# AgatheSenellart/MultiVae

Hardware: AMD Instinct MI355X
Metric: train samples/sec (ELBO step) MoPoE MnistSvhn K=10 (higher is better)
Workload: dtype f32 (error-corrected 2xfp16 / 3xbf16 products, fp32 accumulate); 1 GPU; MoPoE MnistSvhn (mnist MLP + svhn conv), K=10, per-device batch 512, latent_dim 20, Adam lr 1e-3, fwd+ELBO+bwd+optimizer; global_batch=512, K=10, parallelism=dp1, launch=hipGraph replay (fwd + bwd) + Adam

## Files before the change

include/mvk.h:

```cpp
#ifndef MVK_H
#define MVK_H

#include <stdint.h>

#ifdef __cplusplus
extern "C" {
#endif

#define MVK_OK 0
#define MVK_EINVAL (-1)
#define MVK_ELAUNCH (-2)

#define MVK_MAX_MODALITIES 8
#define MVK_MVAE_MAX_SUBSETS 32
#define MVK_IWAE_MAX_EXPERTS 32

#define MVK_DIST_NORMAL 0
#define MVK_DIST_LAPLACE 1
#define MVK_DIST_BERNOULLI 2
#define MVK_DIST_CATEGORICAL 3

#define MVK_ACT_NONE 0
#define MVK_ACT_RELU 1
#define MVK_ACT_SIGMOID 2
// ... 284 lines not shown

int mvk_nchw_to_nhwc(const float* src, float* dst, int n, int c, int h, int w, void* stream);
int mvk_nhwc_to_nchw(const float* src, float* dst, int n, int c, int h, int w, void* stream);

int mvk_poe_fwd(const float* mus, const float* lvs, int E, int64_t n, float eps, int stable, float* mu, float* lv,
                void* stream);
int mvk_poe_bwd(const float* mus, const float* lvs, int E, int64_t n, float eps, int stable, const float* gmu,
                const float* glv, float* dmus, float* dlvs, void* stream);
int mvk_kl_gauss_fwd(const float* mean, int64_t n_mean, const float* lv, int64_t n_lv, const float* pmean, int64_t n_pmean,
                     const float* plv, int64_t n_plv, int64_t rows, int L, float* kl, void* stream);
int mvk_kl_gauss_bwd(const float* mean, int64_t n_mean, const float* lv, int64_t n_lv, const float* pmean, int64_t n_pmean,
                     const float* plv, int64_t n_plv, int64_t rows, int L, const float* g, float* dmean, float* dlv,
                     float* dpmean, float* dplv, void* stream);
int mvk_logprob_fwd(const float* recon, const float* target, int64_t n, int64_t n_target, int dist, float scale, int C,
                    float eps, float* lp, void* stream);
int mvk_logprob_bwd(const float* recon, const float* target, int64_t n, int64_t n_target, int dist, float scale, int C,
                    float eps, const float* g, float* drecon, void* stream);

#define MVK_COPY_MAX 8
typedef struct {
  void* dst;
  const void* src;
  int64_t bytes;
} mvk_copy_desc;
int mvk_copy_batch(const mvk_copy_desc* descs, int n, void* stream);

int mvk_adam_step(float* p, const float* g, float* m, float* v, int64_t n, double lr, double beta1, double beta2,
                  double eps, double weight_decay, int step, double grad_scale, void* stream);
int mvk_adam_step_amsgrad(float* p, const float* g, float* m, float* v, float* vmax, int64_t n, double lr, double beta1,
                          double beta2, double eps, double weight_decay, int step, double grad_scale, void* stream);
int mvk_adam_step_fused(float* p, float* g, float* m, float* v, float* vmax, int64_t n, double lr, double beta1,
                        double beta2, double eps, double weight_decay, int step, double grad_scale, int zero_grad,
                        void* stream);
int mvk_adam_prepare(double* state, float* scalars, void* stream);
int mvk_adam_step_dev(float* p, float* g, float* m, float* v, float* vmax, int64_t n, const float* scalars, int zero_grad,
                      void* stream);
int mvk_adam_step_pub(float* p, float* g, float* m, float* v, float* vmax, int64_t n, double lr, double beta1, double beta2,
                      double eps, double weight_decay, int step, double grad_scale, int zero_grad, float* publish, void* stream);
int mvk_adam_identity(float* scalars, void* stream);

int mvk_heads_fwd(const float* X, const float* W0, const float* b0, float* Y0, const float* W1, const float* b1,
                  float* Y1, int M, int N, int K, int64_t w_sk, int64_t w_sn, void* stream);

int mvk_heads_bwd(const float* X, int x_act, const float* dY0, const float* dY1, const float* W0, const float* W1,
                  int64_t w_sk, int64_t w_sn, int flat_c, float* dX, float* dW0, float* dW1, float* db0, float* db1,
                  float* dbprev, int M, int N, int K, float* ws, int64_t ws_floats, void* stream);

int mvk_defer_begin(float* arena, int64_t arena_floats, const float* grad, int64_t grad_floats);
int mvk_defer_flush(void* stream);
int mvk_defer_end(void* stream);
int64_t mvk_defer_wanted(void);
int mvk_defer_pending(void);

int mvk_comm_id_bytes(void);
int mvk_comm_unique_id(void* id);
int mvk_comm_init(void** comm, int world, int rank, const void* id);
int mvk_comm_destroy(void* comm);
int mvk_allreduce_avg(float* buf, int64_t n, int nseg, void* comm, void* stream);
int mvk_comm_available(void);
int mvk_comm_size(void* comm, int* world, int* rank);
int mvk_allreduce_avg_ranges(float* buf, const int64_t* off, const int64_t* cnt, int nrange, int64_t seg_floats, void* comm,
                             void* stream);
int mvk_event_create(void** ev);
int mvk_event_destroy(void* ev);
int mvk_event_record(void* ev, int external, void* stream);
int mvk_stream_wait_event(void* stream, void* ev);

int mvk_dense16_ok(int M, int N, int K);
int mvk_dense16_pack(const float* W, int N, int K, void* nk_hi, void* nk_lo, float* nk_inv, void* kn_hi, void* kn_lo,
                     float* kn_inv, void* stream);
int mvk_dense16_first(const float* Z, const float* W, const float* bias, const float* z_amax, void* hi, void* lo, float* bound,
                      int M, int N, int K, int act, void* stream);
int mvk_dense16_fwd_nll_rows(int N);
int mvk_dense16_colsum_rows(int M);
int mvk_dense16_fwd_nll(const void* h_hi, const void* h_lo, const float* h_bound, const void* w_hi, const void* w_lo,
                        const float* w_inv, const float* bias, const float* X, int xrows, const float* x_amax, float scale,
                        float grad_weight, void* g_hi, void* g_lo, float* g_bound, float* rows_part, float* colsum_part, int M,
                        int N, int K, void* stream);
int mvk_dense16_bwd_data(const void* g_hi, const void* g_lo, const float* g_bound, const void* wt_hi, const void* wt_lo,
                         const float* wt_inv, const void* mask_hi, float* dA, float* db, float* ws, int64_t ws_floats, int M, int N,
                         int K, void* stream);
int mvk_dense16_wgrad(const void* g_hi, const void* g_lo, const float* g_bound, const void* h_hi, const void* h_lo,
                      const float* h_bound, const float* colsum_part, int cs_rows, float* dW, float* db, float* ws,
                      int64_t ws_floats, int M, int N, int K, void* stream);
int mvk_dense16_unsplit(const void* hi, const void* lo, const float* bound, const float* rowf, float rowf_scale, int rowf_tile,
                        int M, int N, float* out, void* stream);
void mvk_dense16_debug(int flags);
void mvk_dense16_debug_stamps(float* four_floats);

int mvk_nexus_aggregate_fwd(const float* const* msgs, const uint8_t* const* masks, const float* keep_in, const float* u,
                            float dropout_rate, int M, int B, int D, float* agg, float* keep_out, void* stream);
int mvk_nexus_aggregate_bwd(const float* keep, const float* g, int M, int B, int D, float* const* dmsgs, void* stream);

int mvk_nexus_top_nll_fwd(const float* const* z, const float* const* r, const uint8_t* const* masks, const int* D,
                          const float* gamma, const int* adapt, int M, int B, float* const* rows, float* q, float* s2,
                          float* work, void* stream);
int mvk_nexus_top_nll_bwd(const float* const* z, const float* const* r, const uint8_t* const* masks, const int* D,
                          const float* gamma, const int* adapt, int M, int B, const float* const* grows, const float* q,
                          const float* s2, float* work, float* const* dr, void* stream);

int mvk_prof_enable(void* device_slots, int nslots, int32_t* host_kinds, double* host_work);
int mvk_prof_count(void);
int mvk_prof_calibrate(void* device_ticks, int n, void* stream);
int mvk_prof_clock_khz(void);

void mvk_debug_set_phase_buffer(unsigned long long* device_counters);
// ... 7 lines not shown
```

multivae_amd/_lib.py:

```python
import ctypes as C
import os

import torch

_HERE = os.path.dirname(os.path.abspath(__file__))


_ALWAYS_READ = {"MVK_TUNE", "MVK_LIB_PATH", "MVK_DEFER_MB", "MVK_SYNC_DEBUG", "MVK_TRAINER_ALLOW_CPU", "MVK_CPU_THREADS",
                "MVK_BENCH_SAME_GPU", "MVK_FORCE_DIST", "MVK_DIST_BACKEND", "MVK_ADAM_ZERO", "MVK_RCCL", "MVK_BENCH_CHILD", "MVK_OVERLAP", "MVK_GRAPH_ADAM"}


def _warn_ignored_switches():
    if os.environ.get("MVK_TUNE") == "1":
        return
    ignored = sorted(k for k in os.environ if k.startswith("MVK_") and k not in _ALWAYS_READ)
    if ignored:
        import warnings

        warnings.warn(f"{', '.join(ignored)} set without MVK_TUNE=1: experiment switches are ignored unless MVK_TUNE=1 "
                      "(this process runs the shipped configuration)", RuntimeWarning, stacklevel=3)


_warn_ignored_switches()

# ... 70 lines not shown
    "mvk_loss_backward_seed": [C.POINTER(SeedDesc), _i, _p, _p],
    "mvk_f32_to_bf3": [_p, _i64, _p, _p],
    "mvk_bf3_to_f32": [_p, _i64, _p, _p],
    "mvk_conv4s2_small_up_fwd_nll": [_p, _p, _p, _p, _i, _f, _p, _p, _i, _i, _i, _i, _i, _i, _p],
    "mvk_conv4s2_small_up_fwd_nll_w": [_p, _p, _p, _p, _i, _f, _f, _p, _p, _i, _i, _i, _i, _i, _i, _p],
    "mvk_conv4s2_small_up_fwd_nll_s": [_p, _p, _p, _p, _i, _f, _f, _p, _p, _i, _i, _i, _i, _i, _i, _p, _p],
    "mvk_conv4s2_small_up_fwd_s": [_p, _p, _p, _p, _i, _i, _i, _i, _i, _i, _p, _p],
    "mvk_conv4s2_small_up_fwd_nll_sy": [_p, _p, _p, _p, _i, _f, _f, _p, _p, _i, _i, _i, _i, _i, _i, _p, _p, _p],
    "mvk_conv4s2_small_up_bwd_pre_s": [_p, _p, _p, _i, _p, _p, _p, _p, _p, _p, _i64, _i, _i, _i, _i, _i, _p, _p, _p, _p],
    "mvk_conv4s2_small_up_bwd_pre": [_p, _p, _p, _i, _p, _p, _p, _p, _p, _p, _i64, _i, _i, _i, _i, _i, _p],
    "mvk_conv3x3": [_p, _p, _p, _p, _i, _i, _i, _i, _i, _i, _p, _i, _p, _p, _i64, _p],
    "mvk_conv3x3_y": [_p, _p, _p, _p, _i, _i, _i, _i, _i, _i, _p, _i, _p, _p, _p, _i64, _p],
    "mvk_conv3x3_res": [_p, _p, _p, _p, _i, _i, _i, _i, _i, _i, _p, _i, _p, _f, _p, _i64, _p],
    "mvk_conv3x3_wgrad": [_p, _p, _p, _i, _i, _i, _i, _i, _p, _i64, _p],
    "mvk_conv3x3_f": [_p, _p, _p, _p, _i, _i, _i, _i, _i, _i, _p, _i, _p, _f, _p, _i, _f, _p, _i64, _p],
    "mvk_conv3x3_wgrad_f": [_p, _p, _p, _p, _i, _i, _i, _i, _i, _i, _f, _p, _i64, _p],
    "mvk_conv3x3_s": [_p, _p, _p, _p, _i, _i, _i, _i, _i, _i, _p, _i, _p, _f, _p, _i, _f, _p, _p, _p, _p, _i64, _p],
    "mvk_conv3x3_s2": [_p, _p, _p, _p, _p, _i, _i, _i, _i, _i, _i, _p, _f, _p, _p, _p, _p, _i64, _p],
    "mvk_conv3x3_s_part": [_p, _i, _i, _p, _p, _p, _i, _i, _i, _i, _i, _i, _p, _i, _p, _i, _i, _f, _p, _p, _p, _p],
    "mvk_amax": [_p, _i64, _p, _p],
    "mvk_conv4s2_wgrad_s": [_p, _p, _p, _i, _i, _i, _i, _i, _p, _p, _p, _i64, _p],
    "mvk_gemm_smallk_amax": [_p, _p, _p, _i, _i, _i, _i, _p, _i, _i, _p, _p],
    "mvk_conv4s2_small_up_bwd_pre_y": [_p, _p, _p, _i, _p, _p, _p, _p, _p, _p, _i64, _i, _i, _i, _i, _i, _p, _p],
    "mvk_conv4s2_down_s": [_p, _p, _p, _p, _i, _i, _i, _i, _i, _i, _p, _i, _p, _p, _p, _p, _p, _i64, _p, _p],
    "mvk_conv4s2_up_s": [_p, _p, _p, _p, _i, _i, _i, _i, _i, _i, _p, _i, _p, _p, _p, _p, _p, _i64, _p, _p],
    "mvk_conv3x3_wgrad_s": [_p, _p, _p, _p, _i, _i, _i, _i, _i, _i, _f, _p, _p, _p, _i64, _p],
    "mvk_avgpool3s2_fwd": [_p, _p, _i, _i, _i, _i, _p],
    "mvk_avgpool3s2_bwd": [_p, _p, _i, _i, _i, _i, _p],
    "mvk_upsample2_fwd": [_p, _p, _i, _i, _i, _i, _p],
    "mvk_upsample2_bwd": [_p, _p, _i, _i, _i, _i, _p],
    "mvk_axpby": [_p, _f, _p, _f, _i64, _i, _p, _p],
    "mvk_transpose_act": [_p, _p, _i, _i, _i, _i, _p, _i, _p],
    "mvk_probe_mfma_bf16": [_p, _i, _i, _p],
    "mvk_probe_stream_copy": [_p, _p, _i64, _p],
    "mvk_device_rng": [_p, _i64, _p, _i, _f, _f, _p],
    "mvk_conv4s2_wgrad": [_p, _p, _p, _i, _i, _i, _i, _i, _i, _p, _i, _p, _i64, _p],
    "mvk_conv4s2_wgrad_pair": [_p, _p, _p, _i, _i, _i, _i, _p, _p, _p, _i, _i, _i, _i, _i, _p, _i64, _p],
    "mvk_conv4s2_up_nchw_small": [_p, _p, _p, _p, _i, _i, _i, _i, _i, _i, _p],
    "mvk_conv4s2_small_up_fwd": [_p, _p, _p, _p, _i, _i, _i, _i, _i, _i, _p],
    "mvk_conv4s2_small_down_fwd": [_p, _p, _p, _p, _i, _i, _i, _i, _i, _i, _p],
    "mvk_conv4s2_small_down_fwd_wref": [_p, _p, _p, _p, _i, _i, _i, _i, _i, _i, _p],
    "mvk_conv4s2_small_up_bwd": [_p, _p, _i, _p, _i, _p, _p, _p, _p, _p, _p, _i64, _i, _i, _i, _i, _i, _p],
    "mvk_pack_unflatten_weight": [_p, _i, _i, _p, _p],
    "mvk_unflatten_wgrad": [_p, _p, _p, _i, _i, _i, _p, _i64, _p],
    "mvk_flatten_wgrad": [_p, _p, _p, _i, _i, _i, _p, _i64, _p],
    "mvk_nchw_to_nhwc": [_p, _p, _i, _i, _i, _i, _p],
    "mvk_nhwc_to_nchw": [_p, _p, _i, _i, _i, _i, _p],
    "mvk_adam_step": [_p, _p, _p, _p, _i64, _d, _d, _d, _d, _d, _i, _d, _p],
    "mvk_heads_fwd": [_p, _p, _p, _p, _p, _p, _p, _i, _i, _i, _i64, _i64, _p],
    "mvk_heads_bwd": [_p, _i, _p, _p, _p, _p, _i64, _i64, _i, _p, _p, _p, _p, _p, _p, _i, _i, _i, _p, _i64, _p],
    "mvk_defer_begin": [_p, _i64, _p, _i64],
    "mvk_defer_flush": [_p],
    "mvk_defer_end": [_p],
    "mvk_adam_step_amsgrad": [_p, _p, _p, _p, _p, _i64, _d, _d, _d, _d, _d, _i, _d, _p],
    "mvk_adam_step_fused": [_p, _p, _p, _p, _p, _i64, _d, _d, _d, _d, _d, _i, _d, _i, _p],
    "mvk_copy_batch": [C.POINTER(CopyDesc), _i, _p],
    "mvk_adam_prepare": [_p, _p, _p],
    "mvk_adam_step_pub": [_p, _p, _p, _p, _p, _i64, _d, _d, _d, _d, _d, _i, _d, _i, _p, _p],
    "mvk_adam_identity": [_p, _p],
    "mvk_adam_step_dev": [_p, _p, _p, _p, _p, _i64, _p, _i, _p],
    "mvk_mmvae_std_fwd": [_p, _i, _i, _i, _p, _p],
    "mvk_mmvae_std_bwd": [_p, _p, _p, _i, _i, _i, _p, _p],
    "mvk_mmvae_latent_fwd": [_p, _p, _p, _p, _p, _p, _i, _i, _i, _i, _i, _p, _p, _p, _p, _i, _p, _p],
    "mvk_mmvae_objective_fwd": [_p, _p, _p, _p, _i, _i, _i, _i, _p, _p, _p, _p, _p, _f, _p],
    "mvk_mmvae_latent_bwd": [_p, _p, _p, _p, _p, _p, _p, _p, _p, _p, _p, _i, _i, _i, _i, _i, _i, _p, _p, _p, _p, _i, _f, _p],
    "mvk_mmvaeplus_cross_latent_fwd": [_p, _p, _p, _i64, _i, _i, _i, _p, _p],
    "mvk_mmvaeplus_cross_latent_bwd": [_p, _p, _i64, _i, _i, _i, _p, _p, _p],
    "mvk_mvae_posterior_fwd": [_p, _p, _p, _i, _p, _i, _p, _i, _i, _p, _p, _p, _p, _p],
    "mvk_mvae_posterior_bwd": [_p, _p, _p, _i, _p, _i, _p, _p, _i, _i, _p, _p, _p, _p],
    "mvk_gauss_sample_kl_fwd": [_p, _p, _p, _i, _i, _i, _p, _p, _p],
    "mvk_gauss_sample_kl_bwd": [_p, _p, _p, _p, _p, _i, _i, _i, _p, _p, _p],
    "mvk_iwae_sample": [_p, _p, _p, _i, _i, _i, _i, _p, _p],
    "mvk_iwae_logw": [_p, _p, _i, _p, _p, _i, _p, _p, _i, _i, _i, _i, _p, _p],
    "mvk_iwae_reduce": [_p, _i, _i, _i, _p, _p],
    "mvk_poe_fwd": [_p, _p, _i, _i64, _f, _i, _p, _p, _p],
    "mvk_poe_bwd": [_p, _p, _i, _i64, _f, _i, _p, _p, _p, _p, _p],
    "mvk_kl_gauss_fwd": [_p, _i64, _p, _i64, _p, _i64, _p, _i64, _i64, _i, _p, _p],
    "mvk_kl_gauss_bwd": [_p, _i64, _p, _i64, _p, _i64, _p, _i64, _i64, _i, _p, _p, _p, _p, _p, _p],
    "mvk_logprob_fwd": [_p, _p, _i64, _i64, _i, _f, _i, _f, _p, _p],
    "mvk_logprob_bwd": [_p, _p, _i64, _i64, _i, _f, _i, _f, _p, _p, _p],
    "mvk_comm_unique_id": [_p],
    "mvk_comm_init": [C.POINTER(C.c_void_p), _i, _i, _p],
    "mvk_comm_destroy": [_p],
    "mvk_allreduce_avg": [_p, _i64, _i, _p, _p],
    "mvk_comm_size": [_p, C.POINTER(C.c_int), C.POINTER(C.c_int)],
    "mvk_allreduce_avg_ranges": [_p, C.POINTER(C.c_int64), C.POINTER(C.c_int64), _i, _i64, _p, _p],
    "mvk_event_create": [C.POINTER(C.c_void_p)],
    "mvk_event_destroy": [_p],
    "mvk_event_record": [_p, _i, _p],
    "mvk_stream_wait_event": [_p, _p],
    "mvk_dense16_pack": [_p, _i, _i, _p, _p, _p, _p, _p, _p, _p],
    "mvk_dense16_first": [_p, _p, _p, _p, _p, _p, _p, _i, _i, _i, _i, _p],
    "mvk_dense16_fwd_nll": [_p, _p, _p, _p, _p, _p, _p, _p, _i, _p, _f, _f, _p, _p, _p, _p, _p, _i, _i, _i, _p],
    "mvk_dense16_bwd_data": [_p, _p, _p, _p, _p, _p, _p, _p, _p, _p, _i64, _i, _i, _i, _p],
    "mvk_dense16_wgrad": [_p, _p, _p, _p, _p, _p, _p, _i, _p, _p, _p, _i64, _i, _i, _i, _p],
    "mvk_dense16_unsplit": [_p, _p, _p, _p, _f, _i, _i, _i, _p, _p],
    "mvk_nexus_aggregate_fwd": [_p, _p, _p, _p, _f, _i, _i, _i, _p, _p, _p],
    "mvk_nexus_aggregate_bwd": [_p, _p, _i, _i, _i, _p, _p],
    "mvk_nexus_top_nll_fwd": [_p, _p, _p, _p, _p, _p, _i, _i, _p, _p, _p, _p, _p],
    "mvk_nexus_top_nll_bwd": [_p, _p, _p, _p, _p, _p, _i, _i, _p, _p, _p, _p, _p, _p],
}

_lib = None


class MvkError(RuntimeError):
# ... 165 lines not shown
```

multivae_amd/csrc/igemm.hip:

```cpp
#include "igemm_bf.hpp"
#include <mutex>
#include <vector>

namespace mvk {
namespace {
struct DeferState {
  std::mutex mu;
  bool active = false;
  float* arena = nullptr;
  long long cap = 0, used = 0;
  long long wanted = 0;
  const char* g0 = nullptr;
  const char* g1 = nullptr;
  std::vector<DeferItem> items;
  std::vector<hipStream_t> streams;
  std::vector<hipEvent_t> events;
};
DeferState g_defer;

void defer_note_stream(hipStream_t s) {
  for (hipStream_t t : g_defer.streams)
    if (t == s) return;
  g_defer.streams.push_back(s);
}
// ... 93 lines not shown
      it.blk0 = blocks;
      T.it[T.n++] = defer_compact(it);
      const int per = (256 >> it.zl_bits) * (it.vec4 ? 4 : 1);
      blocks += (unsigned)(((long long)it.M * it.N + per - 1) / per);
    }
    hipLaunchKernelGGL(splitk_reduce_batch_kernel, dim3(blocks), dim3(256), 0, s, T);
    if (hipGetLastError() != hipSuccess) rc = MVK_ELAUNCH;
  }
  g_defer.items.clear();
  if (last)
    g_defer.used = 0;
  else
    defer_note_stream(s);
  return rc;
}

extern "C" int mvk_defer_flush(void* stream) {
  std::lock_guard<std::mutex> lock(mvk::g_defer.mu);
  if (!mvk::g_defer.active) return MVK_OK;
  return defer_flush_locked(mvk_stream(stream), false);
}

extern "C" int mvk_defer_end(void* stream) {
  std::lock_guard<std::mutex> lock(mvk::g_defer.mu);
  if (!mvk::g_defer.active) return MVK_OK;
  const int rc = defer_flush_locked(mvk_stream(stream), true);
  mvk::g_defer.active = false;
  return rc;
}

extern "C" int64_t mvk_defer_wanted(void) {
  std::lock_guard<std::mutex> lock(mvk::g_defer.mu);
  return (int64_t)mvk::g_defer.wanted;
}

extern "C" int mvk_defer_pending(void) {
  std::lock_guard<std::mutex> lock(mvk::g_defer.mu);
  return (int)mvk::g_defer.items.size();
}

#include <cstdlib>

namespace mvk {

template <int BM, int BN>
static int launch_cfg(const GemmDesc& d, int zdim, hipStream_t s) {
  dim3 grid((d.M + BM - 1) / BM, (d.N + BN - 1) / BN, zdim);
  hipLaunchKernelGGL((igemm_kernel<BM, BN>), grid, dim3(256), 0, s, d);
  MVK_CHECK_LAUNCH();
  return MVK_OK;
}

static thread_local int g_last_bm = 0;

template <int BM, int BN, int BKT, int AMODE, int BMODE, bool AACT>
static int launch_fast_cfg(const GemmDesc& d, int zdim, hipStream_t s) {
  g_last_bm = BM;
  dim3 grid((d.M + BM - 1) / BM, (d.N + BN - 1) / BN, zdim);
  hipLaunchKernelGGL((igemm_fast_kernel<BM, BN, BKT, AMODE, BMODE, AACT>), grid, dim3(256), 0, s, d);
  MVK_CHECK_LAUNCH();
  return MVK_OK;
}

template <int BM, int BN, int BKT>
static int launch_fast_tile(const GemmDesc& d, int zdim, hipStream_t s, int amode, int bmode, bool aact) {
  if (amode == AM_PLAIN_K && bmode == BM_K && !aact) return launch_fast_cfg<BM, BN, BKT, AM_PLAIN_K, BM_K, false>(d, zdim, s);
  if (amode == AM_PLAIN_K && bmode == BM_N && !aact) return launch_fast_cfg<BM, BN, BKT, AM_PLAIN_K, BM_N, false>(d, zdim, s);
  if (amode == AM_PLAIN_K && bmode == BM_N && aact) return launch_fast_cfg<BM, BN, BKT, AM_PLAIN_K, BM_N, true>(d, zdim, s);
  if (amode == AM_PLAIN_R && bmode == BM_N && !aact) return launch_fast_cfg<BM, BN, BKT, AM_PLAIN_R, BM_N, false>(d, zdim, s);
  if (amode == AM_PLAIN_R && bmode == BM_N && aact) return launch_fast_cfg<BM, BN, BKT, AM_PLAIN_R, BM_N, true>(d, zdim, s);
  if (amode == AM_ROW && bmode == BM_N && !aact) return launch_fast_cfg<BM, BN, BKT, AM_ROW, BM_N, false>(d, zdim, s);
  if (amode == AM_COL && bmode == BM_N && !aact) return launch_fast_cfg<BM, BN, BKT, AM_COL, BM_N, false>(d, zdim, s);
  return 1;
}

template <int BM, int BN, int AMODE, int BMODE, bool AACT>
static int launch_bf_cfg(const GemmDesc& d, int zdim, hipStream_t s) {
  g_last_bm = BM;
  dim3 grid((d.M + BM - 1) / BM, (d.N + BN - 1) / BN, zdim);
  constexpr int DEPTH = 2;
  hipLaunchKernelGGL((igemm_bf_kernel<BM, BN, AMODE, BMODE, AACT, DEPTH>), grid, dim3(256), 0, s, d);
  MVK_CHECK_LAUNCH();
  return MVK_OK;
}

template <int BM, int BN>
static int launch_bf_tile(const GemmDesc& d, int zdim, hipStream_t s, int amode, int bmode, bool aact) {
  if (BM * BN > 128 * 64) {
    if (amode == AM_COL && bmode == BM_N && !aact) return launch_bf_cfg<BM, BN, AM_COL, BM_N, false>(d, zdim, s);
    return 1;
  }
  if (amode == AM_PLAIN_K && bmode == BM_K && !aact) return launch_bf_cfg<BM, BN, AM_PLAIN_K, BM_K, false>(d, zdim, s);
  if (amode == AM_PLAIN_K && bmode == BM_N && !aact) return launch_bf_cfg<BM, BN, AM_PLAIN_K, BM_N, false>(d, zdim, s);
  if (amode == AM_PLAIN_K && bmode == BM_N && aact) return launch_bf_cfg<BM, BN, AM_PLAIN_K, BM_N, true>(d, zdim, s);
  if (amode == AM_PLAIN_R && bmode == BM_N && !aact) return launch_bf_cfg<BM, BN, AM_PLAIN_R, BM_N, false>(d, zdim, s);
  if (amode == AM_PLAIN_R && bmode == BM_N && aact) return launch_bf_cfg<BM, BN, AM_PLAIN_R, BM_N, true>(d, zdim, s);
  if (amode == AM_ROW && bmode == BM_N && !aact) return launch_bf_cfg<BM, BN, AM_ROW, BM_N, false>(d, zdim, s);
  if (amode == AM_COL && bmode == BM_N && !aact) return launch_bf_cfg<BM, BN, AM_COL, BM_N, false>(d, zdim, s);
  if (amode == AM_ROW3 && bmode == BM_N && !aact) return launch_bf_cfg<BM, BN, AM_ROW3, BM_N, false>(d, zdim, s);
  return 1;
}

static int bf_min_blocks() {
  static int v = -1;
  if (v < 0) {
    const char* e = mvk_tune("MVK_BF_MIN_BLOCKS");
    v = e ? atoi(e) : 256;
  }
  return v;
}

static int g_engine = -1;
static int engine() {
  if (g_engine < 0) {
    const char* e = getenv("MVK_ENGINE");
    g_engine = (e && e[0] == 'f') ? 0 : 1;
  }
  return g_engine;
}

static int try_launch_fast(const GemmDesc& d, int zdim, hipStream_t s) {
  const AOperand& A = d.a;
  const long long lim = 1ll << 29;
  if (A.kind == A_PLAIN) {
    if ((long long)d.M * d.K >= lim) return 1;
  } else if ((long long)d.a.H * d.a.W * d.a.C * ((long long)d.M / (d.a.OH * d.a.OW > 0 ? d.a.OH * d.a.OW : 1) + 1) >= lim &&
             !d.a.trans) {
    return 1;
  } else if (d.a.trans && (long long)d.a.H * d.a.W * d.a.C * ((long long)d.K / (d.a.OH * d.a.OW > 0 ? d.a.OH * d.a.OW : 1) + 1) >= lim) {
    return 1;
  }
  if ((long long)d.K * d.N >= lim) return 1;
  int amode = 0, bmode = 0;
  const bool aact = A.act_src != nullptr;
  if (A.kind == A_PLAIN) {
    if (!A.vec4) return 1;
    if (aact && !mvk_aligned16(A.act_src)) return 1;
    amode = A.contig_k ? AM_PLAIN_K : AM_PLAIN_R;
  } else if (A.bf3) {
    if (A.trans || !A.contig_k || A.kind == A_DOWN_NCHW || aact || A.C % 32 != 0 || !mvk_aligned16(A.p) ||
        A.plane_bytes % 16 != 0)
      return MVK_EINVAL;
    amode = AM_ROW3;
  } else if (!A.trans && A.vec4 && A.contig_k && A.kind != A_DOWN_NCHW && !aact) {
    amode = AM_ROW;
  } else if (A.trans && A.vec4 && !A.contig_k && A.kind == A_DOWN && !aact) {
    amode = AM_COL;
  } else {
    return 1;
  }
  if (!d.b.vec4) return 1;
  bmode = d.b.contig_k ? BM_K : BM_N;
  if (d.zmode == Z_SPLITK && (d.ksplit_tiles & 1)) return 1;
  const bool c32 = (amode != AM_ROW) || (A.C % 32 == 0);
  const bool c16 = (amode != AM_ROW) || (A.C % 16 == 0);
  if (amode == AM_ROW3 && !d.b.vec4) return MVK_EINVAL;
  if ((engine() == 1 || amode == AM_ROW3) && c32) {
    auto nb = [&](int bm, int bn) { return (long long)((d.M + bm - 1) / bm) * ((d.N + bn - 1) / bn) * zdim; };
    int rc = 1;
    if (d.N <= 32) {
      rc = launch_bf_tile<128, 32>(d, zdim, s, amode, bmode, aact);
    } else if (d.N > 64 && amode == AM_COL && nb(128, 128) >= 384) {
      rc = launch_bf_tile<128, 128>(d, zdim, s, amode, bmode, aact);
    } else if (nb(128, 64) >= bf_min_blocks() || amode == AM_ROW3) {
      rc = launch_bf_tile<128, 64>(d, zdim, s, amode, bmode, aact);
    }
    if (rc != 1) return rc;
  }
  if (amode == AM_ROW3) return MVK_EINVAL;
  if (d.N <= 32) {
    if (c16 && (long long)((d.M + 255) / 256) * zdim >= 512) return launch_fast_tile<256, 32, 16>(d, zdim, s, amode, bmode, aact);
    return c32 ? launch_fast_tile<128, 32, 32>(d, zdim, s, amode, bmode, aact) : 1;
  }
  auto nblk = [&](int bm, int bn) { return (long long)((d.M + bm - 1) / bm) * ((d.N + bn - 1) / bn) * zdim; };
  if (d.N > 64 && c16 && nblk(128, 128) >= 384) return launch_fast_tile<128, 128, 16>(d, zdim, s, amode, bmode, aact);
  if (!c32) return 1;
  if (nblk(128, 64) >= 384) return launch_fast_tile<128, 64, 32>(d, zdim, s, amode, bmode, aact);
  return launch_fast_tile<64, 64, 32>(d, zdim, s, amode, bmode, aact);
}

static unsigned long long* g_dbg = nullptr;
static int g_dbg_flags = 0;
extern "C" void mvk_debug_set_phase_buffer(unsigned long long* p) { g_dbg = p; }
extern "C" void mvk_debug_set_flags(int f) { g_dbg_flags = f; }

int launch_igemm(const GemmDesc& d_in, int zdim, hipStream_t s, LaunchInfo* info) {
  GemmDesc d = d_in;
  if (info) info->bm = 0;
  d.dbg = g_dbg;
  d.dbg_flags = g_dbg_flags;
  if (d.M <= 0 || d.N <= 0 || d.K <= 0) return MVK_OK;
  {
    g_last_bm = 0;
    const int rc = try_launch_fast(d, zdim, s);
    if (rc != 1) {
      if (info) info->bm = g_last_bm;
      return rc;
    }
    d.e.colsum_part = nullptr;
  }
  if (d.N <= 32) return launch_cfg<128, 32>(d, zdim, s);
  if (d.N <= 64) {
    if (d.M <= 64) return launch_cfg<64, 64>(d, zdim, s);
    return launch_cfg<128, 64>(d, zdim, s);
  }
  long long big = (long long)((d.M + 127) / 128) * ((d.N + 127) / 128) * zdim;
  if (big >= 192) return launch_cfg<128, 128>(d, zdim, s);
  long long mid = (long long)((d.M + 127) / 128) * ((d.N + 63) / 64) * zdim;
  if (mid >= 192 || d.M > 4096) return launch_cfg<128, 64>(d, zdim, s);
  return launch_cfg<64, 64>(d, zdim, s);
}

enum { SPLITK_C4 = 1025, SPLITK_LIN = 1026 };
static int splitk_target(int t) {
  static int t1024 = -1, t512 = -1, tc4 = -1, tlin = -1;
  if (t1024 < 0) {
    const char* a = mvk_tune("MVK_SPLITK_TARGET_1024");
    const char* b = mvk_tune("MVK_SPLITK_TARGET_512");
    const char* c = mvk_tune("MVK_SPLITK_TARGET_C4");
    const char* l = mvk_tune("MVK_SPLITK_TARGET_LIN");
    t1024 = a ? atoi(a) : 768;
    t512 = b ? atoi(b) : 512;
    tc4 = c ? atoi(c) : 256;
    tlin = l ? atoi(l) : t1024;
  }
  return t == 1024 ? t1024 : (t == 512 ? t512 : (t == SPLITK_C4 ? tc4 : (t == SPLITK_LIN ? tlin : t)));
}

int launch_splitk(GemmDesc& d, float* ws, long long ws_floats, int target_blocks, hipStream_t s) {
  target_blocks = splitk_target(target_blocks);
  int tm = (d.M + 127) / 128;
  int tn = (d.N <= 32) ? 1 : (d.N + 63) / 64;
  int tiles = tm * tn;
  int ktiles = (d.K + BK - 1) / BK;
  int splits = target_blocks / (tiles > 0 ? tiles : 1);
  if (splits < 1) splits = 1;
  if (splits > ktiles) splits = ktiles;
  d.zmode = Z_SPLITK;
  d.ksplit_tiles = (ktiles + splits - 1) / splits;
  d.ksplit_tiles += d.ksplit_tiles & 1;
  int z = (ktiles + d.ksplit_tiles - 1) / d.ksplit_tiles;
  const long long need = (long long)z * d.M * d.N;
  if (z > 1 && d.e.atomic && d.e.kind != E_UP && d.e.kind != E_UP_NCHW) {
    if (float* dws = defer_scratch(d.e.out, need, s)) {
      d.e.ws = dws;
      const int rc = launch_igemm(d, z, s);
      return rc ? rc : defer_push(d.e, d.M, d.N, z, (long long)d.M * d.N);
    }
  }
  if (z > 1 && ws && ws_floats >= need && d.e.kind != E_UP && d.e.kind != E_UP_NCHW) {
    d.e.ws = ws;
    int rc = launch_igemm(d, z, s);
    if (rc) return rc;
    long long total = (long long)d.M * d.N;
    hipLaunchKernelGGL(splitk_reduce_kernel, dim3((unsigned)((total + 31) / 32)), dim3(256), 0, s, d.e, d.M, d.N, z);
    MVK_CHECK_LAUNCH();
    return MVK_OK;
  }
  d.e.ws = nullptr;
  return launch_igemm(d, z, s);
}

static void plain_a(AOperand& a, const float* p, long long sr, long long sk, int M, int K) {
  a = AOperand{};
  a.p = p;
  a.kind = A_PLAIN;
  a.sr = sr;
  a.sk = sk;
  a.contig_k = (sk == 1);
  if (sk == 1)
    a.vec4 = (sr % 4 == 0) && (K % 4 == 0) && mvk_aligned16(p);
  else
    a.vec4 = (sr == 1) && (sk % 4 == 0) && (M % 4 == 0) && mvk_aligned16(p);
  a.C = a.H = a.W = a.OH = a.OW = 1;
}

static void plain_b(BOperand& b, const float* p, long long sk, long long sn, int K, int N) {
  b = BOperand{};
  b.p = p;
  b.sk = sk;
  b.sn = sn;
  b.contig_k = (sk == 1);
  if (sk == 1)
    b.vec4 = (sn % 4 == 0) && (K % 4 == 0) && mvk_aligned16(p);
  else
    b.vec4 = (sn == 1) && (sk % 4 == 0) && (N % 4 == 0) && mvk_aligned16(p);
}

static void rowmajor_epi(Epilogue& e, float* out, long long ld) {
  e = Epilogue{};
  e.out = out;
  e.kind = E_ROWMAJOR;
  e.ld = ld;
  e.bias_mod = 1;
  e.Cu = e.OH = e.OW = 1;
}

template <int VEC>
__global__ __launch_bounds__(256) void colsum_kernel(const float* __restrict__ dY, const float* __restrict__ Y, int act,
                                                     int M, int N, int rows_per_block, float* __restrict__ db,
                                                     float* __restrict__ part) {
  const int ncg = (N + VEC - 1) / VEC;
  const int cg_per_blk = ncg < 256 ? ncg : 256;
  const int lanes_r = 256 / cg_per_blk;
  const int cg = blockIdx.x * cg_per_blk + (threadIdx.x % cg_per_blk);
  const int rl = threadIdx.x / cg_per_blk;
// ... 1053 lines not shown
```

multivae_amd/csrc/igemm.hpp:

```cpp
#pragma once
#include "common.hpp"

namespace mvk {

enum AKind { A_PLAIN = 0, A_DOWN = 1, A_DOWN_NCHW = 2, A_UP = 3 };
enum EpiKind { E_ROWMAJOR = 0, E_UP = 1, E_CONVREF = 2, E_UNFLATREF = 3, E_UP_NCHW = 4 };
enum ZMode { Z_NONE = 0, Z_SPLITK = 1, Z_PARITY = 2 };

struct AOperand {
  const float* p;
  int kind;
  int trans;
  long long sr, sk;
  int contig_k;
  int vec4;
  int C, H, W;
  int OH, OW;
  const float* act_src;
  int act;
  int tw, mul;
  int bf3;
  long long plane_bytes;
};

struct BOperand {
  const float* p;
  long long sk, sn;
  int contig_k;
  int vec4;
  long long z_stride;
};

struct Epilogue {
  float* out;
  int kind;
  long long ld;
  const float* bias;
  int bias_mod;
  int act;
  const float* act_src;
  int src_act;
  int atomic;
  int Cu, OH, OW;
  int taps;
  float* ws;
  float* colsum_part;
  const float* res;
  float res_alpha;
};

struct GemmDesc {
  AOperand a;
  BOperand b;
  Epilogue e;
  int M, N, K;
  int zmode;
  int ksplit_tiles;
  unsigned long long* dbg;
  int dbg_flags;
};

constexpr int MIN_WAVES = 3;
constexpr int BK = 16;

template <int BM, int BN>
struct TileCfg {
  static constexpr int WAVES_N = (BN >= 64) ? 2 : 1;
  static constexpr int WAVES_M = 4 / WAVES_N;
  static constexpr int WTM = BM / WAVES_M;
  static constexpr int WTN = BN / WAVES_N;
  static constexpr int TM = WTM / 32;
  static constexpr int TN = WTN / 32;
  static constexpr int SA = BM + 4;
  static constexpr int SB = BN + 4;
  static constexpr int NA1 = BM * BK / 256;
  static constexpr int NB1 = BN * BK / 256;
  static constexpr int NA4 = (BM * BK / 4 + 255) / 256;
  static constexpr int NB4 = (BN * BK / 4 + 255) / 256;
  static constexpr int NA = (4 * NA4 > NA1) ? 4 * NA4 : NA1;
  static constexpr int NB = (4 * NB4 > NB1) ? 4 * NB4 : NB1;
  static constexpr int UA4 = BM * BK / 4;
  static constexpr int UB4 = BN * BK / 4;
  static_assert(TM >= 1 && TN >= 1, "tile too small");
};

typedef float f32x16 __attribute__((ext_vector_type(16)));

struct Pos {
  int n, i, j;
};
__device__ __forceinline__ Pos decode_pos(int pos, int OH, int OW) {
  Pos p;
  p.j = pos % OW;
  int t = pos / OW;
  p.i = t % OH;
  p.n = t / OH;
  return p;
}

__device__ __forceinline__ int a_mul(const AOperand& a) { return a.mul > 0 ? a.mul : 2; }
__device__ __forceinline__ void a_tap(const AOperand& a, int tap, int& kh, int& kw) {
// ... 704 lines not shown
  }
  red[zl][e] = v;
  __syncthreads();
  if (zl != 0 || idx >= total) return;
  v = ((red[0][e] + red[1][e]) + (red[2][e] + red[3][e])) + ((red[4][e] + red[5][e]) + (red[6][e] + red[7][e]));
  splitk_store(E, N, idx, v);
}

template <int V>
__device__ __forceinline__ void splitk_reduce_bodyv(const Epilogue& E, int M, int N, int nz, long long zstride,
                                                    unsigned block, int zl_bits, float* red ) {
  const int ZL = 1 << zl_bits, EL = 256 >> zl_bits;
  const int e = threadIdx.x & (EL - 1);
  const int zl = threadIdx.x >> (8 - zl_bits);
  const long long total = (long long)M * N;
  const long long idx = ((long long)block * EL + e) * V;
  float v[V];
#pragma unroll
  for (int c = 0; c < V; ++c) v[c] = 0.f;
  if (idx < total) {
#pragma unroll 8
    for (int z = zl; z < nz; z += ZL) {
      const float* src = E.ws + (long long)z * zstride + idx;
      if (V == 4) {
        const float4 t = *reinterpret_cast<const float4*>(src);
        v[0] += t.x;
        v[1 % V] += t.y;
        v[2 % V] += t.z;
        v[3 % V] += t.w;
      } else {
        v[0] += *src;
      }
    }
  }
  const int ld = EL * V + 1;
#pragma unroll
  for (int c = 0; c < V; ++c) red[zl * ld + e * V + c] = v[c];
  __syncthreads();
  if (zl != 0 || idx >= total) return;
#pragma unroll
  for (int c = 0; c < V; ++c) {
    float acc = 0.f;
    for (int g = 0; g < ZL; g += 8) {
      const float* r = red + g * ld + e * V + c;
      acc += ((r[0] + r[ld]) + (r[2 * ld] + r[3 * ld])) + ((r[4 * ld] + r[5 * ld]) + (r[6 * ld] + r[7 * ld]));
    }
    splitk_store(E, N, idx + c, acc);
  }
}

__global__ __launch_bounds__(256) void splitk_reduce_kernel(const Epilogue E, int M, int N, int nz) {
  __shared__ float red[8][33];
  splitk_reduce_body(E, M, N, nz, (long long)M * N, blockIdx.x, red);
}

struct DeferItem {
  Epilogue e;
  int M, N, nz;
  unsigned blk0;
  long long zstride;
  int vec4;
  int zl_bits;
};
struct DeferItemC {
  float* out;
  const float* ws;
  const float* bias;
  const float* act_src;
  long long ld, zstride;
  int M, N, nz;
  unsigned blk0;
  int Cu, bias_mod;
  short kind, act, src_act, taps;
  unsigned char atomic, vec4, zl_bits, pad;
};
constexpr int DEFER_BATCH = 40;
struct DeferTable {
  int n;
  DeferItemC it[DEFER_BATCH];
};
static_assert(sizeof(DeferTable) <= 4096, "kernel-argument limit");
inline DeferItemC defer_compact(const DeferItem& d) {
  DeferItemC c{};
  c.out = d.e.out, c.ws = d.e.ws, c.bias = d.e.bias, c.act_src = d.e.act_src;
  c.ld = d.e.ld, c.zstride = d.zstride;
  c.M = d.M, c.N = d.N, c.nz = d.nz, c.blk0 = d.blk0;
  c.Cu = d.e.Cu, c.bias_mod = d.e.bias_mod;
  c.kind = (short)d.e.kind, c.act = (short)d.e.act, c.src_act = (short)d.e.src_act, c.taps = (short)d.e.taps;
  c.atomic = (unsigned char)d.e.atomic, c.vec4 = (unsigned char)d.vec4, c.zl_bits = (unsigned char)d.zl_bits;
  return c;
}
__global__ __launch_bounds__(256) void splitk_reduce_batch_kernel(const DeferTable T) {
  __shared__ float red[32 * 33];
  int i = 0;
  for (int j = 1; j < T.n; ++j)
    if (blockIdx.x >= T.it[j].blk0) i = j;
  const DeferItemC& it = T.it[i];
  Epilogue E{};
  E.out = it.out, E.ws = const_cast<float*>(it.ws), E.bias = it.bias, E.act_src = it.act_src;
  E.ld = it.ld, E.Cu = it.Cu, E.bias_mod = it.bias_mod;
  E.kind = it.kind, E.act = it.act, E.src_act = it.src_act, E.taps = it.taps, E.atomic = it.atomic;
  if (it.vec4)
    splitk_reduce_bodyv<4>(E, it.M, it.N, it.nz, it.zstride, blockIdx.x - it.blk0, it.zl_bits, red);
  else
    splitk_reduce_bodyv<1>(E, it.M, it.N, it.nz, it.zstride, blockIdx.x - it.blk0, it.zl_bits, red);
}
// ... 36 lines not shown
```

multivae_amd/csrc/igemm_bf.hpp:

```cpp
#pragma once
#include "bf3.hpp"
#include "igemm_fast.hpp"

namespace mvk {

constexpr int BF_OCC_SMALL = 3;

template <int BM, int BN>
struct BfCfg {
  static constexpr int BKT = 32;
  static constexpr int WAVES_N = (BN >= 64) ? 2 : 1;
  static constexpr int WAVES_M = 4 / WAVES_N;
  static constexpr int WTM = BM / WAVES_M;
  static constexpr int WTN = BN / WAVES_N;
  static constexpr int TM = WTM / 32;
  static constexpr int TN = WTN / 32;
  static constexpr int RS = 80;
  static constexpr int GA = (BM / 4) * RS + 64;
  static constexpr int GB = (BN / 4) * RS + 64;
  static constexpr int A_PIECE = 4 * GA;
  static constexpr int B_PIECE = 4 * GB;
  static constexpr int LDS_BYTES = 3 * (A_PIECE + B_PIECE);
  static constexpr int NA4 = BM * BKT / 4 / 256;
  static constexpr int NB4 = BN * BKT / 4 / 256;
// ... 399 lines not shown
            bfr[b][p] = *reinterpret_cast<const bf16x8*>(b_frag + p * T::B_PIECE + b * 8 * 80 + ks * 32);
#pragma unroll
        for (int q = 0; q < 6; ++q) {
#pragma unroll
          for (int a = 0; a < T::TM; ++a)
#pragma unroll
            for (int b = 0; b < T::TN; ++b)
              acc[a][b] = __builtin_amdgcn_mfma_f32_32x32x16_bf16(af[a][PA[q]], bfr[b][PB[q]], acc[a][b], 0, 0, 0);
          const int slot = ks * 6 + q;
          convert_range(slot * NPAIR / NSLOT, (slot + 1) * NPAIR / NSLOT, ra, ya, rb);
        }
      }
    }
    MVK_T(0)
    __syncthreads();
    MVK_T(1)
    write_pieces(ra);
    MVK_T(2)
    __syncthreads();
    MVK_T(3)
  };

#pragma unroll
  for (int i = 0; i < DEPTH; ++i) load_tiles(kbeg + i * BKT, ra[i], ya[i], rb[i]);
  convert_range(0, NPAIR, ra[0], ya[0], rb[0]);
  write_pieces(ra[0]);
  __syncthreads();
  int t = 0;
  for (; t + DEPTH <= ntiles; t += DEPTH) {
#pragma unroll
    for (int i = 0; i < DEPTH; ++i) {
      load_tiles(kbeg + (t + i + DEPTH) * BKT, ra[i], ya[i], rb[i]);
      __builtin_amdgcn_sched_barrier(0);
      step(ra[(i + 1) % DEPTH], ya[(i + 1) % DEPTH], rb[(i + 1) % DEPTH]);
    }
  }
#pragma unroll
  for (int i = 0; i < DEPTH - 1; ++i)
    if (t + i < ntiles) step(ra[(i + 1) % DEPTH], ya[(i + 1) % DEPTH], rb[(i + 1) % DEPTH]);
  if (T::TM * T::TN == 1) {
#pragma unroll
    for (int r = 0; r < 16; ++r) acc[0][0][r] += acc2[r];
  }
#ifdef MVK_PHASES
  if (d.dbg && lane == 0) {
    for (int i = 0; i < 4; ++i) atomicAdd(d.dbg + i, tphase[i]);
    atomicAdd(d.dbg + 5, (unsigned long long)ntiles);
    atomicAdd(d.dbg + 7, 1ull);
  }
#endif
  float* lds = reinterpret_cast<float*>(lds_raw);
  if (run_epilogue_vec<T, BM, BN, T::LDS_BYTES / 4>(d, acc, lds, tid, m0, n0, wm, wn, l31, lhi, ph, pw)) return;
  run_epilogue<T>(d, acc, lds, tid, m0, n0, wm, wn, l31, lhi, ph, pw, (int)bid_z);
}

template <int BM, int BN, int AMODE, int BMODE, bool AACT, int DEPTH>
__global__ __launch_bounds__(256, (BM * BN <= 128 * 32) ? BF_OCC_SMALL : ((BM * BN <= 128 * 64) ? 3 : 2)) void igemm_bf_kernel(const GemmDesc d) {
  igemm_bf_body<BM, BN, AMODE, BMODE, AACT, DEPTH>(d, blockIdx.x, blockIdx.y, blockIdx.z);
}

template <int BM, int BN, int AMODE, int BMODE, bool AACT, int DEPTH>
__global__ __launch_bounds__(256, (BM * BN <= 128 * 32) ? BF_OCC_SMALL : ((BM * BN <= 128 * 64) ? 3 : 2)) void igemm_bf_pair_kernel(
    const GemmDesc d0, const GemmDesc d1, const unsigned n0, const unsigned gx0, const unsigned gy0, const unsigned gx1,
    const unsigned gy1) {
  unsigned b = blockIdx.x;
  if (b < n0) {
    igemm_bf_body<BM, BN, AMODE, BMODE, AACT, DEPTH>(d0, b % gx0, (b / gx0) % gy0, b / (gx0 * gy0));
  } else {
    b -= n0;
    igemm_bf_body<BM, BN, AMODE, BMODE, AACT, DEPTH>(d1, b % gx1, (b / gx1) % gy1, b / (gx1 * gy1));
  }
}

}
```

multivae_amd/schedule.py:

```python
import ctypes as C
import os

import torch

from . import _lib
from ._lib import call, ptr, stream_ptr

_WS = {}
_ARENA = {}
_ARENA_RETIRED = []
_ARENA_CAPTURED = set()
_SIDE = {}
_CONST_ROWS = {}
_TERMS_WS = {}

_OPEN = {}
scope = _OPEN.get

WS_FLOATS = 16 * 1024 * 1024


def _ws(like):
    key = (like.device, torch.cuda.current_stream(like.device).cuda_stream)
    t = _WS.get(key)
    if t is None:
        t = torch.empty(WS_FLOATS, dtype=torch.float32, device=like.device)
        _WS[key] = t
    return t


def _side_stream(device, i):
    key = (device, i)
    st = _SIDE.get(key)
    if st is None:
        st = _lib.new_stream(device)
        _SIDE[key] = st
    return st


def const_rows(device, n, value):
    key = (device, int(n), float(value))
    t = _CONST_ROWS.get(key)
    if t is None:
        if torch.cuda.is_current_stream_capturing():
            return None
        t = torch.full((int(n),), float(value), dtype=torch.float32, device=device)
        _CONST_ROWS[key] = t
    return t


def terms_workspace(device, stream=None):
    key = (device, (torch.cuda.current_stream(device) if stream is None else stream).cuda_stream)
    ws = _TERMS_WS.get(key)
    if ws is None and not torch.cuda.is_current_stream_capturing():
        ws = _TERMS_WS[key] = torch.zeros(1 + 32 * 64, dtype=torch.float32, device=device)
    return ws


def swap_arena(device, arena):
    old = _ARENA.pop(device, None)
    if arena is not None:
        _ARENA[device] = arena
    return old


def _tensors_of(obj):
    if torch.is_tensor(obj):
        yield obj
    elif isinstance(obj, dict):
        for v in obj.values():
            yield from _tensors_of(v)
    elif isinstance(obj, (list, tuple)):
        for v in obj:
            yield from _tensors_of(v)


DEFER = _lib.tune("MVK_DEFER", "1") != "0"
DEFER_ARENA_CAP_FLOATS = int(os.environ.get("MVK_DEFER_MB", "1024")) * (1 << 18)
DEFER_ARENA_START_FLOATS = min(64 * (1 << 18), DEFER_ARENA_CAP_FLOATS)

# ... 329 lines not shown
```

multivae_amd/trainers/graph.py:

```python
import os

import torch

from .. import _lib, kernels, schedule
from ..data.datasets.base import DatasetOutput


class GraphedStep:
    def __init__(self, model, flat, inputs, noise=None, warmup=3, capture_error_mode="global", optimizer=None, overlap=False,
                 rotate=None, **fwd_kwargs):
        dev = flat.flat.device
        if dev.type != "cuda":
            raise RuntimeError("GraphedStep needs a GPU")
        self.model, self.flat, self.fwd_kwargs = model, flat, fwd_kwargs
        if rotate is not None and (optimizer is not None or overlap or not hasattr(rotate, "set_rotation")):
            raise ValueError("GraphedStep(rotate=...) excludes optimizer= / overlap= and needs a trainers.FusedAdam")
        self.rot_opt = rotate
        self.rotation = schedule.Rotation(dev) if rotate is not None else None
        self.rotated = False
        self.optimizer = optimizer if (optimizer is not None and getattr(optimizer, "zero_grad_in_step", False)
                                       and hasattr(optimizer, "step_captured") and not overlap) else None
        self.includes_optimizer = self.optimizer is not None
        self.overlap_point = schedule.OverlapPoint(dev) if overlap else None
        self.early_ranges = self.late_ranges = None
        if self.optimizer is not None:
            self.optimizer.sync_device_state()
        self._seed = None
        self.data = {m: v.detach().clone() for m, v in inputs.data.items()}
        extra = {}
        if hasattr(inputs, "masks"):
            self.masks = {m: v.detach().clone() for m, v in inputs.masks.items()}
            extra["masks"] = self.masks
        else:
            self.masks = None
        self.inputs = DatasetOutput(data=self.data, **extra)
        self.noise = self._clone(noise)
        prof = kernels.PROFILE.pop("recon_nll", None)
        try:
            cur = torch.cuda.current_stream(dev)
            side = schedule._side_stream(dev, 62)
            side.wait_stream(cur)
            with torch.cuda.stream(side):
                for _ in range(max(int(warmup), 2 if self.rotation is not None else 1)):
                    self.flat.zero_grad()
                    self._body()
                if self.rotation is not None:
                    self.flat.zero_grad()
            cur.wait_stream(side)
            torch.cuda.synchronize(dev)
            if self.rotation is not None:
                ranges = flat.ranges_of(self.rotation.params)
                if ranges:
                    self.rot_opt.set_rotation(ranges)
                    self.rotated = True
                else:
                    self.rotation = None
            for st in (cur, schedule._side_stream(dev, 30)):
                schedule.terms_workspace(dev, st)
            self.graph = torch.cuda.CUDAGraph()
            with torch.cuda.graph(self.graph, capture_error_mode=capture_error_mode):
                self.out = self._body(capture=True)
            op = self.overlap_point
            if op is not None and op.recorded:
                self.late_ranges = flat.ranges_of(op.late_params, strict=True)
                self.early_ranges = flat.complement(self.late_ranges) if self.late_ranges else None
                if not self.early_ranges:
                    self.early_ranges = self.late_ranges = None
        finally:
            if prof is not None:
                kernels.PROFILE["recon_nll"] = prof

    @staticmethod
    def _clone(noise):
        if noise is None:
            return None
        if isinstance(noise, dict):
            return {k: v.detach().clone() for k, v in noise.items()}
        return noise.detach().clone()

    def _body(self, capture=False):
        kw = dict(self.fwd_kwargs)
        if self.noise is not None:
            kw["noise"] = self.noise
        opt = self.optimizer if capture else None
        rot = self.rotation
        step = schedule.deferred_reductions(self.flat, prelude=opt.prepare_captured if opt is not None else None,
                                            overlap=self.overlap_point, rotation=rot)
        try:
            with step:
                if rot is not None:
                    rot.begin_step(self.rot_opt.rot_update if (capture and self.rotated) else None)
                out = self.model(self.inputs, **kw)
                out.loss.backward(gradient=kernels.unit_seed(out.loss))
            if opt is not None:
                step.run_prelude()
                opt.step_captured()
        finally:
            if rot is not None:
                rot.end_step()
        return out

    def matches(self, inputs):
        return (set(inputs.data.keys()) == set(self.data.keys())
                and all(inputs.data[m].shape == self.data[m].shape for m in self.data)
                and (hasattr(inputs, "masks") == (self.masks is not None)))

    def __call__(self, inputs=None, noise=None):
        if inputs is not None and inputs is not self.inputs:
            pairs = [(self.data[m], v) for m, v in inputs.data.items() if v is not self.data[m]]
            if self.masks is not None:
                pairs += [(self.masks[m], v) for m, v in inputs.masks.items() if v is not self.masks[m]]
            self._copy_in(pairs)
        if noise is not None and self.noise is not None:
# ... 57 lines not shown
```

Baseline: 541,200 samples/s.

## Fuse split-K reduction into GEMM tail via atomic ticket counters

Adds per-tile ticket counters so the last-arriving split-K slice of each output tile performs the reduction and epilogue store. This removes the separate splitk_reduce_kernel launch for bf GEMMs without colsum/residual epilogues. A two-level reduction handles more than 8 slices. The cost is extra atomic fences, serialization at the last block, and counter buffers registered before graph capture.

```diff
diff --git a/include/mvk.h b/include/mvk.h
--- a/include/mvk.h
+++ b/include/mvk.h
@@ -360,6 +360,8 @@
 int64_t mvk_defer_wanted(void);
 int mvk_defer_pending(void);
 
+int mvk_splitk_tickets(const float* ws, unsigned* counters, int64_t count);
+
 int mvk_comm_id_bytes(void);
 int mvk_comm_unique_id(void* id);
 int mvk_comm_init(void** comm, int world, int rank, const void* id);
diff --git a/multivae_amd/_lib.py b/multivae_amd/_lib.py
--- a/multivae_amd/_lib.py
+++ b/multivae_amd/_lib.py
@@ -146,6 +146,7 @@
     "mvk_defer_begin": [_p, _i64, _p, _i64],
     "mvk_defer_flush": [_p],
     "mvk_defer_end": [_p],
+    "mvk_splitk_tickets": [_p, _p, _i64],
     "mvk_adam_step_amsgrad": [_p, _p, _p, _p, _p, _i64, _d, _d, _d, _d, _d, _i, _d, _p],
     "mvk_adam_step_fused": [_p, _p, _p, _p, _p, _i64, _d, _d, _d, _d, _d, _i, _d, _i, _p],
     "mvk_copy_batch": [C.POINTER(CopyDesc), _i, _p],
diff --git a/multivae_amd/csrc/igemm.hip b/multivae_amd/csrc/igemm.hip
--- a/multivae_amd/csrc/igemm.hip
+++ b/multivae_amd/csrc/igemm.hip
@@ -169,6 +169,7 @@
 }
 
 static thread_local int g_last_bm = 0;
+static thread_local bool g_last_fin = false;
 
 template <int BM, int BN, int BKT, int AMODE, int BMODE, bool AACT>
 static int launch_fast_cfg(const GemmDesc& d, int zdim, hipStream_t s) {
@@ -194,6 +195,7 @@
 template <int BM, int BN, int AMODE, int BMODE, bool AACT>
 static int launch_bf_cfg(const GemmDesc& d, int zdim, hipStream_t s) {
   g_last_bm = BM;
+  g_last_fin = d.e.ws && d.e.tickets;
   dim3 grid((d.M + BM - 1) / BM, (d.N + BN - 1) / BN, zdim);
   constexpr int DEPTH = 2;
   hipLaunchKernelGGL((igemm_bf_kernel<BM, BN, AMODE, BMODE, AACT, DEPTH>), grid, dim3(256), 0, s, d);
@@ -218,7 +220,13 @@
   return 1;
 }
 
+static unsigned long long* g_dbg = nullptr;
+static int g_dbg_flags = 0;
+constexpr int FIN_OFF = 0x1000;
+constexpr int BF_ANY = 0x2000;
+
 static int bf_min_blocks() {
+  if (g_dbg_flags & BF_ANY) return 0;
   static int v = -1;
   if (v < 0) {
     const char* e = mvk_tune("MVK_BF_MIN_BLOCKS");
@@ -296,10 +304,37 @@
   return launch_fast_tile<64, 64, 32>(d, zdim, s, amode, bmode, aact);
 }
 
-static unsigned long long* g_dbg = nullptr;
-static int g_dbg_flags = 0;
 extern "C" void mvk_debug_set_phase_buffer(unsigned long long* p) { g_dbg = p; }
 extern "C" void mvk_debug_set_flags(int f) { g_dbg_flags = f; }
+
+namespace {
+struct TicketBlock {
+  const float* ws;
+  unsigned* cnt;
+  long long n;
+};
+std::mutex g_tickets_mu;
+std::vector<TicketBlock> g_tickets;
+}
+static unsigned* tickets_for(const float* ws, long long need) {
+  if (!ws || (g_dbg_flags & FIN_OFF)) return nullptr;
+  std::lock_guard<std::mutex> lock(g_tickets_mu);
+  for (const TicketBlock& b : g_tickets)
+    if (b.ws == ws) return need <= b.n ? b.cnt : nullptr;
+  return nullptr;
+}
+
+extern "C" int mvk_splitk_tickets(const float* ws, unsigned* counters, int64_t count) {
+  if (!ws || (counters && count <= 0)) return MVK_EINVAL;
+  std::lock_guard<std::mutex> lock(g_tickets_mu);
+  for (size_t i = 0; i < g_tickets.size(); ++i)
+    if (g_tickets[i].ws == ws) {
+      g_tickets.erase(g_tickets.begin() + i);
+      break;
+    }
+  if (counters) g_tickets.push_back({ws, counters, (long long)count});
+  return MVK_OK;
+}
 
 int launch_igemm(const GemmDesc& d_in, int zdim, hipStream_t s, LaunchInfo* info) {
   GemmDesc d = d_in;
@@ -367,8 +402,12 @@
   }
   if (z > 1 && ws && ws_floats >= need && d.e.kind != E_UP && d.e.kind != E_UP_NCHW) {
     d.e.ws = ws;
+    d.e.fin_nz = z;
+    d.e.tickets = (d.e.colsum_part || d.e.res) ? nullptr : tickets_for(ws, 9ll * tm * ((d.N + 31) / 32));
+    g_last_fin = false;
     int rc = launch_igemm(d, z, s);
     if (rc) return rc;
+    if (g_last_fin) return MVK_OK;
     long long total = (long long)d.M * d.N;
     hipLaunchKernelGGL(splitk_reduce_kernel, dim3((unsigned)((total + 31) / 32)), dim3(256), 0, s, d.e, d.M, d.N, z);
     MVK_CHECK_LAUNCH();
diff --git a/multivae_amd/csrc/igemm.hpp b/multivae_amd/csrc/igemm.hpp
--- a/multivae_amd/csrc/igemm.hpp
+++ b/multivae_amd/csrc/igemm.hpp
@@ -47,6 +47,8 @@
   float* colsum_part;
   const float* res;
   float res_alpha;
+  unsigned* tickets;
+  int fin_nz;
 };
 
 struct GemmDesc {
@@ -857,6 +859,59 @@
 __global__ __launch_bounds__(256) void splitk_reduce_kernel(const Epilogue E, int M, int N, int nz) {
   __shared__ float red[8][33];
   splitk_reduce_body(E, M, N, nz, (long long)M * N, blockIdx.x, red);
+}
+
+__device__ __forceinline__ bool splitk_arrive(unsigned* cnt, unsigned full, unsigned* flag) {
+  asm volatile("s_waitcnt vmcnt(0)" ::: "memory");
+  __syncthreads();
+  if (threadIdx.x == 0) {
+    __builtin_amdgcn_fence(__ATOMIC_RELEASE, "agent");
+    asm volatile("s_waitcnt vmcnt(0)" ::: "memory");
+    const unsigned t = __hip_atomic_fetch_add(cnt, 1u, __ATOMIC_RELAXED, __HIP_MEMORY_SCOPE_AGENT);
+    if (t == full - 1) {
+      __hip_atomic_store(cnt, 0u, __ATOMIC_RELAXED, __HIP_MEMORY_SCOPE_AGENT);
+      __builtin_amdgcn_fence(__ATOMIC_ACQUIRE, "agent");
+      asm volatile("s_waitcnt vmcnt(0)" ::: "memory");
+    }
+    *flag = t;
+  }
+  __syncthreads();
+  const bool last = *flag == full - 1;
+  __syncthreads();
+  return last;
+}
+
+__device__ __forceinline__ void splitk_finish_tile(const GemmDesc& d, int m0, int n0, int BM, int BN, unsigned tile, unsigned z,
+                                                   unsigned* flag) {
+  const Epilogue& E = d.e;
+  const int nz = E.fin_nz;
+  unsigned* cnt = E.tickets + 9 * (size_t)tile;
+  const int rows = (d.M - m0) < BM ? (d.M - m0) : BM, cols = (d.N - n0) < BN ? (d.N - n0) : BN;
+  const int count = rows * cols;
+  const long long MN = (long long)d.M * d.N;
+  const int l = z & 7;
+  if (nz > 8) {
+    if (!splitk_arrive(cnt + 1 + l, (unsigned)(nz - l + 7) / 8, flag)) return;
+    for (int i = threadIdx.x; i < count; i += 256) {
+      const int r = i / cols;
+      float* p = E.ws + (long long)(m0 + r) * d.N + n0 + (i - r * cols);
+      float v = 0.f;
+#pragma unroll 4
+      for (int zz = l; zz < nz; zz += 8) v += __hip_atomic_load(p + zz * MN, __ATOMIC_RELAXED, __HIP_MEMORY_SCOPE_AGENT);
+      __hip_atomic_store(p + l * MN, v, __ATOMIC_RELAXED, __HIP_MEMORY_SCOPE_AGENT);
+    }
+  }
+  const int groups = nz < 8 ? nz : 8;
+  if (!splitk_arrive(cnt, (unsigned)groups, flag)) return;
+  for (int i = threadIdx.x; i < count; i += 256) {
+    const int r = i / cols;
+    const long long idx = (long long)(m0 + r) * d.N + n0 + (i - r * cols);
+    float p[8];
+#pragma unroll
+    for (int g = 0; g < 8; ++g)
+      p[g] = g < groups ? 0.f + __hip_atomic_load(E.ws + g * MN + idx, __ATOMIC_RELAXED, __HIP_MEMORY_SCOPE_AGENT) : 0.f;
+    splitk_store(E, d.N, idx, ((p[0] + p[1]) + (p[2] + p[3])) + ((p[4] + p[5]) + (p[6] + p[7])));
+  }
 }
 
 struct DeferItem {
diff --git a/multivae_amd/csrc/igemm_bf.hpp b/multivae_amd/csrc/igemm_bf.hpp
--- a/multivae_amd/csrc/igemm_bf.hpp
+++ b/multivae_amd/csrc/igemm_bf.hpp
@@ -475,6 +475,8 @@
   float* lds = reinterpret_cast<float*>(lds_raw);
   if (run_epilogue_vec<T, BM, BN, T::LDS_BYTES / 4>(d, acc, lds, tid, m0, n0, wm, wn, l31, lhi, ph, pw)) return;
   run_epilogue<T>(d, acc, lds, tid, m0, n0, wm, wn, l31, lhi, ph, pw, (int)bid_z);
+  if (d.e.ws && d.e.tickets)
+    splitk_finish_tile(d, m0, n0, BM, BN, bid_x + bid_y * ((d.M + BM - 1) / BM), bid_z, reinterpret_cast<unsigned*>(lds_raw));
 }
 
 template <int BM, int BN, int AMODE, int BMODE, bool AACT, int DEPTH>
diff --git a/multivae_amd/schedule.py b/multivae_amd/schedule.py
--- a/multivae_amd/schedule.py
+++ b/multivae_amd/schedule.py
@@ -7,6 +7,7 @@
 from ._lib import call, ptr, stream_ptr
 
 _WS = {}
+_WS_TICKETS = {}
 _ARENA = {}
 _ARENA_RETIRED = []
 _ARENA_CAPTURED = set()
@@ -18,6 +19,7 @@
 scope = _OPEN.get
 
 WS_FLOATS = 16 * 1024 * 1024
+WS_TICKETS = 16 * 1024
 
 
 def _ws(like):
@@ -26,6 +28,9 @@
     if t is None:
         t = torch.empty(WS_FLOATS, dtype=torch.float32, device=like.device)
         _WS[key] = t
+    if key not in _WS_TICKETS and not torch.cuda.is_current_stream_capturing():
+        tk = _WS_TICKETS[key] = torch.zeros(WS_TICKETS, dtype=torch.int32, device=like.device)
+        call("mvk_splitk_tickets", ptr(t), ptr(tk), tk.numel())
     return t
 
 
diff --git a/multivae_amd/trainers/graph.py b/multivae_amd/trainers/graph.py
--- a/multivae_amd/trainers/graph.py
+++ b/multivae_amd/trainers/graph.py
@@ -58,7 +58,10 @@
             for st in (cur, schedule._side_stream(dev, 30)):
                 schedule.terms_workspace(dev, st)
             self.graph = torch.cuda.CUDAGraph()
-            with torch.cuda.graph(self.graph, capture_error_mode=capture_error_mode):
+            capture = torch.cuda.graph(self.graph, capture_error_mode=capture_error_mode)
+            with torch.cuda.stream(capture.capture_stream):
+                schedule._ws(self.flat.flat)
+            with capture:
                 self.out = self._body(capture=True)
             op = self.overlap_point
             if op is not None and op.recorded:
```

New measurement: 461,300 samples/s. -14.8%, worse.
